# LemonATsu/UNet-PhaseGen

Hardware: AMD Instinct MI355X
Metric: spectrogram-frames/sec (train fwd+bwd) (higher is better)
Workload: dtype f32; 1 GPU; train.py full step (fwd + cos/sin/mag loss + bwd + Adam), UNetModel(1024, 2048), per-GPU batch 64 x 1024 bins x 256 frames (BASELINE configs[2]); global_batch=64, frames=256, channels=1024, parallelism=dp1, grad_allreduce_payload=fp32, adam=fused into the wgrad epilogues

## Files before the change

### unet-phasegen_amd/csrc/conv_common.h

```cpp
#pragma once
#include <hip/hip_runtime.h>
#include <stdint.h>
#include "phasegen.h"
#include "pg_common.h"

namespace pgconv {

struct IgemmParams {
    const float* x; long x_bs;
    const float* w;
    const float* pt; long pt_bs;
    float* y; long y_bs;
    const float* add; long add_bs;
    const float* ref; long ref_bs;
    unsigned x_bytes, w_bytes, pt_bytes;
    int B, Q, M, Lx, Ly, k, s, p;
    int act_x, act_p, mask_mode;
    int U, u_off;
    int LP; float inv_LP;
    int a_vec;
    int tilesM, tilesN;
    int g_ps;
    int tn_stride;
    float* y2; long y2_bs; float y_slope, y2_slope;
    float* ws;
    int nslab;
    int whole;
    int sr;
    int n_lo;
    int x_pitch;
    unsigned short* yh; long yh_bs; int yh_pitch; float yh_slope;
    unsigned short* yh2; long yh2_bs; int yh2_pitch; float yh2_slope;
    float* ad_p; float* ad_m; float* ad_v; PgAdamScalars ad;
    const float* qk; unsigned qk_bytes; int qk_bs, Lq;
    const float* pk; unsigned pk_bytes; int Kp;
};

}
using pgconv::IgemmParams;

namespace {


constexpr int WMB = 4;
constexpr int BM = 64 * WMB, BN = 128, BK = 16, NT = 256;
constexpr int TILE_A = BM * BK, TILE_B = BN * BK;
constexpr int STAGE = TILE_A + TILE_B;
constexpr int AE = BM / 16;

typedef float f32x16 __attribute__((ext_vector_type(16)));


typedef __amdgpu_buffer_rsrc_t rsrc_t;
constexpr int OOB = 0x7ffffff0;
__device__ __forceinline__ rsrc_t make_rsrc(const float* p, unsigned bytes) {
    return __builtin_amdgcn_make_buffer_rsrc(const_cast<float*>(p), 0, (int)bytes, 0x00020000);
}
__device__ __forceinline__ float bload(rsrc_t r, int elem_off, bool ok) {
    return __builtin_bit_cast(float, __builtin_amdgcn_raw_buffer_load_b32(r, ok ? elem_off * 4 : OOB, 0, 0));
}

__device__ __forceinline__ int xcd_remap(int bid, int nwg) {
    const int xcd = bid & 7, local = bid >> 3, q = nwg >> 3, r = nwg & 7;
    return (xcd < r ? xcd * (q + 1) : r * (q + 1) + (xcd - r) * q) + local;
}

template <int MB, int NB> struct AccT { f32x16 c[MB][NB]; };
using Acc = AccT<WMB, 2>;
using AccR = AccT<2, 4>;

__device__ __forceinline__ int dma_kt(int lane, int w) { return ((((lane >> 2) & 3) ^ w) << 2) | (lane & 3); }
__device__ __forceinline__ int dma_row(int lane, int w, int e) { return 16 * e + 4 * w + (lane >> 4); }

__device__ __forceinline__ int dma16_row(int lane, int w, int e) { return (4 * e + w) * 16 + (lane >> 2); }
__device__ __forceinline__ int dma16_kc(int lane) { return ((lane & 3) ^ ((lane >> 4) & 3)) << 2; }
#ifndef PG_ABL
#define PG_ABL 0
#endif
#if PG_ABL == 4
#define PG_ADDR(x) ((x) & 0x3f0)
#else
#define PG_ADDR(x) (x)
#endif
__device__ __forceinline__ void dma16(rsrc_t r, float* lds_wave_uniform, int byte_off) {
    __builtin_amdgcn_raw_ptr_buffer_load_lds(r, lds_wave_uniform, 16, PG_ADDR(byte_off), 0, 0, 0);
}
__device__ __forceinline__ void dma4(rsrc_t r, float* lds_wave_uniform, int byte_off) {
    __builtin_amdgcn_raw_ptr_buffer_load_lds(r, lds_wave_uniform, 4, PG_ADDR(byte_off), 0, 0, 0);
}
__device__ __forceinline__ void dma4s(rsrc_t r, float* lds_wave_uniform, int lane_off, int uniform_off) {
    __builtin_amdgcn_raw_ptr_buffer_load_lds(r, lds_wave_uniform, 4, lane_off, uniform_off, 0, 0);
}
__device__ __forceinline__ void dma16s(rsrc_t r, float* lds_wave_uniform, int lane_off, int uniform_off) {
    __builtin_amdgcn_raw_ptr_buffer_load_lds(r, lds_wave_uniform, 16, lane_off, uniform_off, 0, 0);
}

typedef __bf16 bf16x8 __attribute__((ext_vector_type(8)));
__device__ __forceinline__ bf16x8 to_bf16x8(float v0, float v1, float v2, float v3, float v4, float v5, float v6, float v7) {
    bf16x8 r;
    r[0] = (__bf16)v0; r[1] = (__bf16)v1; r[2] = (__bf16)v2; r[3] = (__bf16)v3;
    r[4] = (__bf16)v4; r[5] = (__bf16)v5; r[6] = (__bf16)v6; r[7] = (__bf16)v7;
    return r;
}
__device__ __forceinline__ bf16x8 to_bf16x8(const f32x4 (&v)[2]) { return to_bf16x8(v[0][0], v[0][1], v[0][2], v[0][3], v[1][0], v[1][1], v[1][2], v[1][3]); }
__device__ __forceinline__ bf16x8 to_bf16x8(const float (&v)[8]) { return to_bf16x8(v[0], v[1], v[2], v[3], v[4], v[5], v[6], v[7]); }
template <int MB, int NB>
__device__ __forceinline__ void mfma_bf16(const bf16x8 (&A)[MB], const bf16x8 (&B)[NB], AccT<MB, NB>& acc) {
#pragma unroll
    for (int i = 0; i < MB; ++i)
#pragma unroll
        for (int j = 0; j < NB; ++j) acc.c[i][j] = __builtin_amdgcn_mfma_f32_32x32x16_bf16(A[i], B[j], acc.c[i][j], 0, 0, 0);
}
typedef float f32x2 __attribute__((ext_vector_type(2)));
typedef __bf16 bf16x2 __attribute__((ext_vector_type(2)));
typedef unsigned u32x4 __attribute__((ext_vector_type(4)));
__device__ __forceinline__ void split_bf16(const float (&v)[8], bf16x8& hi, bf16x8& lo) {
    u32x4 H, L;
#pragma unroll
    for (int i = 0; i < 4; ++i) {
        const f32x2 x = {v[2 * i], v[2 * i + 1]};
        const bf16x2 h = __builtin_convertvector(x, bf16x2);
        const unsigned P = __builtin_bit_cast(unsigned, h);
// ... 363 lines not shown
```

### unet-phasegen_amd/csrc/conv_igemm.hip

```cpp
#include <hip/hip_runtime.h>
#include <cstring>
#include <cmath>
#include <algorithm>
#include "conv_fixup.h"

namespace {

constexpr int WG_PER_CU = 2;
constexpr int MAX_STREAMK_WG = 2048;
constexpr long WS_PER_WG = 2L * ACC_REGS * NT * 4;
constexpr long WS_STREAMK = (long)MAX_STREAMK_WG * WS_PER_WG;

struct Knobs {
    int prec;
    int force_mode;
    int no_raw;
    int no_tall;
    int oversub;
    int contended;
    int no_ps;
    int no_raw3;
    int all_raw3;
    int sr;
    int force_colsplit;
// ... 264 lines not shown
    if (ptrs && (!a->x || !a->w || (!a->y && !a->yh && !a->yh2))) return pg_fail(PG_ERR_NULL, "conv_fwd_h: x, w and at least one output required");
    if (((uintptr_t)a->x & 3) || ((uintptr_t)a->w & 15) || (a->x_bs & 1) || (a->x_pitch & 1))
        return pg_fail(PG_ERR_ALIGN, "conv_fwd_h: x must be 4-byte aligned with even pitch / batch stride, w 16-byte aligned");
    if (a->x_pitch <= a->Lin) return pg_fail(PG_ERR_SHAPE, "conv_fwd_h: x_pitch must exceed Lin (zero tail of at least one element)");
    if ((a->yh && a->yh_pitch < a->Lout) || (a->yh2 && a->yh2_pitch < a->Lout)) return pg_fail(PG_ERR_SHAPE, "conv_fwd_h: output pitch below Lout");
    pg_conv_args kb = {};
    kb.schedule = a->schedule;
    if (int e = decode_knobs(&kb, kn)) return e;
    p = {};
    p.x = reinterpret_cast<const float*>(a->x); p.x_bs = a->x_bs; p.x_pitch = a->x_pitch;
    p.w = reinterpret_cast<const float*>(a->w);
    p.y = a->y; p.y_bs = a->y_bs; p.y_slope = 1.0f; p.y2_slope = 1.0f;
    p.yh = a->yh; p.yh_bs = a->yh_bs; p.yh_pitch = a->yh_pitch; p.yh_slope = pg_act_slope(a->yh_act);
    p.yh2 = a->yh2; p.yh2_bs = a->yh2_bs; p.yh2_pitch = a->yh2_pitch; p.yh2_slope = pg_act_slope(a->yh2_act);
    p.B = a->B; p.Q = a->Cin; p.M = a->Cout; p.Lx = a->Lin; p.Ly = a->Lout; p.k = a->k; p.s = a->stride; p.p = a->pad;
    p.ws = (float*)a->workspace;
    const long xe = ((long)(p.B - 1) * p.x_bs + (long)p.Q * p.x_pitch) * 2;
    if (xe <= 0 || xe >= 0x7ffffff0L) return pg_fail(PG_ERR_SHAPE, "conv_fwd_h: activation tensor exceeds 2 GiB (31-bit buffer offsets)");
    p.x_bytes = (unsigned)xe;
    const int kwp = tr ? pg_shadow_taps(p.k, p.s) : p.k;
    const long wbytes = (long)p.M * (tr ? p.s : 1) * p.Q * kwp * 2;
    if (wbytes >= 0x7ffffff0L) return pg_fail(PG_ERR_SHAPE, "conv_fwd_h: weight shadow exceeds 2 GiB");
    p.w_bytes = (unsigned)wbytes;
    if (tr) {
        p.u_off = p.p / p.s;
        p.U = (p.Ly - 1 + p.p) / p.s - p.u_off + 1;
        if (p.U <= 0) return pg_fail(PG_ERR_SHAPE, "conv_fwd_h: empty output");
    }
    if (!pgconv::h_supported(tr ? KIND_T : KIND_F, p)) return pg_fail(PG_ERR_UNSUPPORTED, "conv_fwd_h: geometry not covered by the bf16-resident kernels (use the fp32-tensor entry points)");
    return PG_OK;
}

int plan_h3(const pg_convh_args* a, ConvPlan& pl) {
    Knobs kn;
    ConvPart& c = pl.main;
    IgemmParams& p = c.p;
    if (int e = h3_params(a, true, p, kn)) return e;
    const bool tr = a->transposed != 0;
    pl.kind = tr ? KIND_T : KIND_F; pl.prec = 0; pl.has_tail = false; pl.pack = 0; c.fam = FAM_H3;
    const long rows = tr ? (long)p.M * p.s : p.M, cols = (long)p.B * (tr ? p.U : p.Ly);
    p.tilesM = (int)((rows + 255) / 256);
    p.tilesN = (int)((cols + 255) / 256);
    p.tn_stride = 256;
    p.nslab = (int)((long)p.Q * (tr ? pg_shadow_taps(p.k, p.s) : p.k) / 32);
    c.tiles = (long)p.tilesM * p.tilesN;
    if (c.tiles <= 0 || c.tiles > 0x0fffffffL || p.nslab <= 0) return pg_fail(PG_ERR_SHAPE, "conv_fwd_h: empty or oversize grid");
    set_grid(c, kn, a->workspace_bytes);
    return PG_OK;
}

hipError_t launch_fixup(const ConvPlan& pl, const ConvPart& c, hipStream_t st) {
    typedef void (*Fn)(const IgemmParams, int);
#define FIX2(KIND, MB, NB, WN) {conv_fixup_kernel<KIND, MB, NB, WN, false>, conv_fixup_kernel<KIND, MB, NB, WN, true>}
    static const Fn table[4][4][2] = {
        {FIX2(FIX_F, WMB, 2, 2), FIX2(FIX_T, WMB, 2, 2), FIX2(FIX_G, WMB, 2, 2), {}},
        {FIX2(FIX_F, 2, 4, 2), FIX2(FIX_T, 2, 4, 2), FIX2(FIX_G, 2, 4, 2), FIX2(FIX_T_PM, 2, 4, 2)},
        {FIX2(FIX_F, 2, 4, 1), FIX2(FIX_T, 2, 4, 1), {}, FIX2(FIX_T_PM, 2, 4, 1)},
        {FIX2(FIX_F, 8, 2, 4), FIX2(FIX_T, 8, 2, 4), {}, {conv_fixup_kernel<FIX_T_PM, 8, 2, 4, false>, nullptr}}};
#undef FIX2
    const int geom = c.fam == FAM_IM2COL ? 0 : (c.fam == FAM_RAW_TALL ? 2 : (c.fam == FAM_RAW3 || c.fam == FAM_H3 ? 3 : 1));
    const bool pm = pl.kind == KIND_T && c.p.s == 2 && (c.fam == FAM_RAW || c.fam == FAM_RAW_TALL || c.fam == FAM_RAW3);
    const bool wide = c.fixup == FIXUP_WIDE;
    const Fn fn = table[geom][pm ? FIX_T_PM : (int)pl.kind][wide];
    if (!fn) return hipErrorInvalidDeviceFunction;
    const long blocks = (c.tiles - c.p.whole) * (geom == 3 ? 16 : 8) * (wide ? 4 : 1);
    hipLaunchKernelGGL(fn, dim3((unsigned)blocks), dim3(NT), 0, st, c.p, c.grid);
    return hipGetLastError();
}

hipError_t part_kernel(const ConvPlan& pl, const ConvPart& c, hipStream_t st, char* name = nullptr) {
    const IgemmParams& p = c.p;
    const Kind kind = pl.kind;
    const char* tk = kind == KIND_T ? "true" : "false";
    hipError_t e = hipSuccess;
    switch (c.fam) {
        case FAM_RAW_TALL:
            if (name) snprintf(name, 96, "conv_raw_kernel<%d, %d, %s, %d, 1>", p.k, p.s, tk, pl.prec);
            else e = pgconv::launch_raw_ft_tall(kind, p, c.grid, st, pl.prec);
            break;
        case FAM_RAW:
            if (name) snprintf(name, 96, "conv_raw_kernel<%d, %d, %s, %d, 2>", p.k, p.s, tk, pl.prec);
            else e = pgconv::launch_raw_ft(kind, p, c.grid, st, pl.prec);
            break;
        case FAM_G_RAW:
        case FAM_G_PS:
            if (name) snprintf(name, 96, "conv_g_%s_kernel<%d, %d, %d>", c.fam == FAM_G_PS ? "ps" : "raw", p.k, p.s, pl.prec);
            else e = pgconv::launch_raw_g(p, c.grid, st, pl.prec);
            break;
        case FAM_IM2COL:
            if (name) snprintf(name, 96, "conv_%c_kernel<0, 0, %d>", "ftg"[kind], pl.prec);
            else e = pgconv::launch_im2col(kind, p, c.grid, st, pl.prec);
            break;
        case FAM_RAW3:
            if (name) snprintf(name, 96, "conv_raw3_kernel<%d, %d, %s, %s>", p.k, p.s, tk, p.act_x == PG_ACT_NONE ? "false" : "true");
            else e = pgconv::launch_raw3(kind, p, c.grid, st);
            break;
        case FAM_H3:
            if (name) snprintf(name, 96, "conv_h3_kernel<%d, %d, %s>", kind == KIND_T && p.k == 5 ? 8 : p.k, p.s, tk);
            else e = pgconv::launch_h3(kind, p, c.grid, st);
            break;
    }
    if (!name && e == hipSuccess && c.fixup != FIXUP_NONE) e = launch_fixup(pl, c, st);
    return e;
}

void describe(const ConvPlan& pl, char* buf, int buflen) {
    static const char* const fixup_name[] = {"none", "plain", "wide"};
    const ConvPart& c = pl.main;
    char name[96];
    (void)part_kernel(pl, c, nullptr, name);
    snprintf(buf, (size_t)buflen, "%s|grid=%d|tiles=%ld|slabs=%d|split=%d|whole=%d|fixup=%s", name, c.grid, c.tiles, c.p.nslab,
             (int)(c.fixup != FIXUP_NONE), c.p.whole, fixup_name[c.fixup]);
    if (!pl.has_tail) return;
// ... 70 lines not shown
```

### unet-phasegen_amd/csrc/conv_raw_wgrad.hip

```cpp
#include "conv_common.h"

namespace {

template <int KW, int S> struct GRaw {
    static constexpr int WL = 15 * S + KW;
    static constexpr int WLP = g_wlp(KW, S);
    static constexpr int NQT = RBN / KW;
    static constexpr int TNV = NQT * KW;
    static constexpr int SUB = NQT * WLP;
    static constexpr int SUBS = (SUB + 63) / 64 * 64;
    static constexpr int NE = (SUB + NT - 1) / NT;
    static constexpr int SUBP = (SUB + 255) / 256 * 256;
    static constexpr int NE16 = (SUB / 4 + NT - 1) / NT;
    static constexpr int STG_FLAT_BF = RTILE_A + 2 * SUBS, STG_FLAT_F32 = RTILE_A + 2 * SUBP, STG_PS = RTILE_A + SUBP;
    static_assert(WL <= WLP, "window does not fit its slot");
    static_assert(WLP % 4 == 0 && WLP <= 64, "16-byte window pieces; channel 0 inside the first 64 floats");
    static_assert(2 * STG_FLAT_F32 * 4 <= 64 * 1024, "LDS budget");
};

#define G_HEAD(STG)                                                                                       \
    __shared__ __attribute__((aligned(16))) float lds[2 * (STG)];                                         \
    const int tid = threadIdx.x, lane = tid & 63;                                                         \
    const int wv = __builtin_amdgcn_readfirstlane(tid >> 6), wm = wv >> 1, wn = wv & 1;

#define G_TILE                                                                                            \
    const int m0 = (tile / p.tilesN) * RBM, n0 = (tile % p.tilesN) * C::TNV;                              \
    const int qbase = (tile % p.tilesN) * C::NQT;

#define G_A_PIECES(PITCH)                                                                                 \
    _Pragma("unroll") for (int e = 0; e < 2; ++e) {                                                       \
        const int m = m0 + dma16_row(lane, wv, e);                                                        \
        pv[e] = m < p.M ? (m * (PITCH) + dma16_kc(lane)) * 4 : FAR;                                       \
    }

#define G_FRAG_BASE_ACC(MORE)                                                                             \
    int bbase[4];                                                                                         \
    _Pragma("unroll") for (int jb = 0; jb < 4; ++jb) {                                                    \
        const int c = wn * 128 + jb * 32 + (lane & 31), qc = c / KW;                                      \
        bbase[jb] = qc * C::WLP + (c - qc * KW) + S * 8 * (lane >> 5);                                    \
        MORE                                                                                              \
    }                                                                                                     \
    AccR acc;                                                                                             \
    _Pragma("unroll") for (int i = 0; i < 2; ++i) _Pragma("unroll") for (int j = 0; j < 4; ++j)           \
        _Pragma("unroll") for (int r = 0; r < 16; ++r) acc.c[i][j][r] = 0.f;

#define G_READ_INTERIOR                                                                                   \
    _Pragma("unroll") for (int i = 0; i < 2; ++i) a[i][0] = *reinterpret_cast<const f32x4*>(ap + i * 32 * BK + (((2 * h) ^ sw) << 2)); \
    _Pragma("unroll") for (int ip = 0; ip < 4; ++ip) {                                                    \
        if (ip == 2) {                                                                                    \
            _Pragma("unroll") for (int i = 0; i < 2; ++i) a[i][1] = *reinterpret_cast<const f32x4*>(ap + i * 32 * BK + (((2 * h + 1) ^ sw) << 2)); \
        }                                                                                                 \
        _Pragma("unroll") for (int jb = 0; jb < 4; ++jb) { b[jb][2 * ip] = Bw[bbase[jb] + S * 2 * ip]; b[jb][2 * ip + 1] = Bw[bbase[jb] + S * (2 * ip + 1)]; } \
    }

#define G_READ_FLAT(SLOT)                                                                                 \
    if (kc_cur >= 16) {                                                                                   \
        G_READ_INTERIOR                                                                                   \
    } else {                                                                                              \
        _Pragma("unroll") for (int c = 0; c < 2; ++c)                                                     \
            _Pragma("unroll") for (int i = 0; i < 2; ++i) a[i][c] = *reinterpret_cast<const f32x4*>(ap + i * 32 * BK + (((2 * h + c) ^ sw) << 2)); \
        typedef const volatile __attribute__((address_space(3))) float* lds_vptr;                         \
        const lds_vptr Bv = (lds_vptr)Bw;                                                                 \
        const int shift = (SLOT) - S * kc_cur;                                                            \
        _Pragma("unroll") for (int i = 0; i < 8; ++i) {                                                   \
            const int d = (8 * h + i >= kc_cur) ? shift : 0;                                              \
            _Pragma("unroll") for (int jb = 0; jb < 4; ++jb) b[jb][i] = Bv[bbase[jb] + S * i + d];        \
        }                                                                                                 \
    }

#define G_ACT                                                                                             \
    if (slopeA != 1.0f) {                                                                                 \
        _Pragma("unroll") for (int i = 0; i < 2; ++i) _Pragma("unroll") for (int c = 0; c < 2; ++c)       \
            _Pragma("unroll") for (int v = 0; v < 4; ++v) a[i][c][v] = pg_act_apply(a[i][c][v], slopeA);  \
    }                                                                                                     \
    if (slopeB != 1.0f) {                                                                                 \
        _Pragma("unroll") for (int jb = 0; jb < 4; ++jb)                                                  \
            _Pragma("unroll") for (int i = 0; i < 8; ++i) b[jb][i] = pg_act_apply(b[jb][i], slopeB);      \
    }

#define G_MFMA(BF)                                                                                        \
    if (BF) mfma_low_2x4<BF>(a, b, acc);                                                                  \
    else {                                                                                                \
        _Pragma("unroll") for (int kk = 0; kk < 8; ++kk)                                                  \
            _Pragma("unroll") for (int i = 0; i < 2; ++i) _Pragma("unroll") for (int j = 0; j < 4; ++j)   \
                acc.c[i][j] = __builtin_amdgcn_mfma_f32_32x32x2f32(a[i][kk >> 2][kk & 3], b[j][kk], acc.c[i][j], 0, 0, 0); \
    }

#if defined(PG_G_ABL) && PG_G_ABL == 1
#define G_ISSUE_NEXT(STG, ISSUE, SKIP) SKIP
#else
#define G_ISSUE_NEXT(STG, ISSUE, SKIP) ISSUE(lds + (cur ^ 1) * (STG), (sl + 1) * BK)
#endif
#if defined(PG_G_ABL) && PG_G_ABL == 2
#define G_BARRIER asm volatile("s_waitcnt lgkmcnt(0)\n\ts_barrier" ::: "memory");
#else
#define G_BARRIER __syncthreads();
#endif

#define G_SLAB_LOOP(STG, BF, ISSUE, SKIP, PRIMED, FRAGS, ADVANCE)                                         \
    PG_STAMP_DECL                                                                                         \
    ISSUE(lds, sb * BK)                                                                                   \
    PRIMED                                                                                                \
    __syncthreads();                                                                                      \
    for (int sl = sb; sl < se; ++sl) {                                                                    \
        const int cur = (sl - sb) & 1;                                                                    \
        PG_STAMP(0)                                                                                       \
        G_ISSUE_NEXT(STG, ISSUE, SKIP)                                                                    \
        __builtin_amdgcn_sched_barrier(0);                                                                \
        PG_STAMP(1)                                                                                       \
        {   const float* As = lds + cur * (STG);                                                          \
            const float* Bw = As + RTILE_A;                                                               \
            const int r = lane & 31, h = lane >> 5, sw = (r >> 2) & 3;                                    \
            const float* ap = As + (wm * 64 + r) * BK;                                                    \
            f32x4 a[2][2];                                                                                \
            float b[4][8];                                                                                \
            FRAGS                                                                                         \
            G_MFMA(BF)                                                                                    \
        }                                                                                                 \
        __builtin_amdgcn_sched_barrier(0);                                                                \
        PG_STAMP(2)                                                                                       \
        ADVANCE                                                                                           \
        G_BARRIER                                                                                         \
        PG_STAMP(3)                                                                                       \
    }                                                                                                     \
    PG_STAMP_FLUSH

#define G_FINISH(G, SLOT)                                                                                 \
    if (sb == 0 && se == p.nslab) epilogue_g<S, 2, 4>(p, acc, m0, n0, lane, wm, wn, n0 + C::TNV);         \
    else store_partial(p.ws, G, SLOT, acc, tid);

#define G_FLAT_START                                                                                      \
    int gb, gi;                                                                                           \
    { const int k0 = sb * BK; gb = k0 / p.LP; gi = k0 - gb * p.LP; }                                      \
    int kc_cur = 16, kc_next;
#define G_FLAT_ISSUED      kc_next = kc < 16 ? kc : 16; gi += BK; if (gi >= p.LP) { gi -= p.LP; ++gb; }
#define G_FLAT_SKIP        kc_next = 16;
#define G_FLAT_ADVANCE     kc_cur = kc_next;
#define G_PS_NEXT(B_, C_)  if (++C_ == cps) { C_ = 0; ++B_; }
#define G_NOTHING

template <int KW, int S, int BF>
__device__ __forceinline__ void g_raw_bf(const IgemmParams& p) {
    using C = GRaw<KW, S>;
    G_HEAD(C::STG_FLAT_BF)
    const int kt = dma_kt(lane, wv);
    const rsrc_t rp = make_rsrc(p.pt, p.pt_bytes), rx = make_rsrc(p.x, p.x_bytes);
    const float slopeA = pg_act_slope(p.act_p), slopeB = pg_act_slope(p.act_x);
    const int pbs4 = (int)p.pt_bs * 4, xbs4 = (int)p.x_bs * 4;
    Walk wk(p);
    while (wk.more()) {
        int tile, sb, se;
        wk.segment(p, tile, sb, se);
        G_TILE

        int aoff[8];
#pragma unroll
        for (int e = 0; e < 8; ++e) {
            const int m = m0 + dma_row(lane, wv, e);
            aoff[e] = m < p.M ? m * p.LP * 4 : FAR;
        }
        constexpr bool RECOMP = KW <= 5 && BF != 0;
        int choff[RECOMP ? 1 : C::NE], vv[RECOMP ? 1 : C::NE];
        if (!RECOMP) {
#pragma unroll
            for (int e = 0; e < C::NE; ++e) {
                const int idx = tid + NT * e, ql = idx / C::WLP, v = idx - ql * C::WLP;
                choff[e] = (idx < C::SUB && qbase + ql < p.Q) ? (qbase + ql) * p.Lx * 4 : FAR;
                vv[e] = v - p.p;
            }
        }
#define GRAW_CHOFF(e) (RECOMP ? ({ int t_ = tid; asm volatile("" : "+v"(t_)); const int idx_ = t_ + NT * (e), ql_ = idx_ / C::WLP; \
                                  (idx_ < C::SUB && qbase + ql_ < p.Q) ? (qbase + ql_) * p.Lx * 4 : FAR; }) : choff[RECOMP ? 0 : (e)])
#define GRAW_VV(e) (RECOMP ? ({ int t_ = tid; asm volatile("" : "+v"(t_)); const int idx_ = t_ + NT * (e); idx_ - (idx_ / C::WLP) * C::WLP - p.p; }) \
                           : vv[RECOMP ? 0 : (e)])
        constexpr bool FASTP = BF != 2 && !(KW <= 5 && BF != 0);
        constexpr bool FASTW = FASTP && KW != 4;
        int pv[FASTP ? 2 : 1], woff[FASTW ? C::NE16 : 1];
        if (FASTW) {
#pragma unroll
            for (int e = 0; e < C::NE16; ++e) {
                const int f = 4 * (tid + NT * e), ql = f / C::WLP, v0 = f - ql * C::WLP;
                woff[e] = (f < C::SUB && qbase + ql < p.Q) ? ((qbase + ql) * p.Lx + v0) * 4 : FAR;
            }
        }
        if (FASTP) { G_A_PIECES(p.LP) }
        G_FRAG_BASE_ACC(G_NOTHING)
        G_FLAT_START

#define GRAW_ISSUE(STAGE_PTR, K0)                                                                         \
    {   float* const As = (STAGE_PTR) + wv * 64; float* const Bw = (STAGE_PTR) + RTILE_A + wv * 64;       \
        const int k0 = (K0);                                                                              \
        const int kc = p.LP - gi;                            \
        if (FASTP && kc >= 16 && gb < p.B) {                                                              \
            const int sa = gb * pbs4 + gi * 4;                                                            \
            _Pragma("unroll") for (int e = 0; e < 2; ++e) dma16s(rp, As + wv * 192 + e * 1024, pv[FASTP ? e : 0], sa); \
        } else {                                                                                          \
          int bb, ii; divmod24(k0 + kt, p.LP, p.inv_LP, bb, ii);                                          \
          const int po = bb < p.B ? bb * pbs4 + ii * 4 : OOB;                                             \
          _Pragma("unroll") for (int e = 0; e < 8; ++e) dma4(rp, As + e * 256, aoff[e] + po); }           \
        const int w0 = S * gi - p.p;                             \
        if (FASTW && kc >= 16 && gb < p.B && w0 >= 0 && w0 + C::WLP <= p.Lx) {    \
            const int sw_ = gb * xbs4 + w0 * 4;                                                           \
            _Pragma("unroll") for (int e = 0; e < C::NE16; ++e)                                           \
                if (4 * (e * NT + wv * 64) < C::SUB) dma16s(rx, (STAGE_PTR) + RTILE_A + 4 * (e * NT + wv * 64), woff[FASTW ? e : 0], sw_); \
        } else {                                                                                          \
        const int sb0 = gb < p.B ? gb * xbs4 : -NEVER, sb1 = (kc < 16 && gb + 1 < p.B) ? (gb + 1) * xbs4 : -NEVER; \
        _Pragma("unroll") for (int e = 0; e < C::NE; ++e) {                                               \
            if ((e + 1) * NT <= C::SUB || e * NT + wv * 64 < C::SUB) {                                    \
                const int ps = S * gi + GRAW_VV(e);                                                       \
                dma4(rx, Bw + e * NT, ((unsigned)ps < (unsigned)p.Lx && sb0 >= 0) ? sb0 + GRAW_CHOFF(e) + ps * 4 : FAR); \
            }                                                                                             \
        }                                                                                                 \
        if (kc < 16) {                                  \
            _Pragma("unroll") for (int e = 0; e < C::NE; ++e) {                                           \
                if ((e + 1) * NT <= C::SUB || e * NT + wv * 64 < C::SUB) {                                                          \
                    const int ps = GRAW_VV(e);                                                            \
                    dma4(rx, Bw + C::SUBS + e * NT, ((unsigned)ps < (unsigned)p.Lx && sb1 >= 0) ? sb1 + GRAW_CHOFF(e) + ps * 4 : FAR); \
                }                                                                                         \
            }                                                                                             \
        }                                                                                                 \
        }                                                                                                 \
        G_FLAT_ISSUED                                                                                     \
    }
#define GRAW_FRAGS G_READ_FLAT(C::SUBS) G_ACT
        G_SLAB_LOOP(C::STG_FLAT_BF, BF, GRAW_ISSUE, G_FLAT_SKIP, G_FLAT_ADVANCE, GRAW_FRAGS, G_FLAT_ADVANCE)
#undef GRAW_FRAGS
#undef GRAW_ISSUE
#undef GRAW_CHOFF
#undef GRAW_VV
        G_FINISH(wk.g, wk.slot)
        wk.next(se - sb);
    }
}

template <int KW, int S, int BF>
__device__ __forceinline__ void g_ps_bf(const IgemmParams& p) {
    using C = GRaw<KW, S>;
    G_HEAD(C::STG_PS)
    const rsrc_t rp = make_rsrc(p.pt, p.pt_bytes), rx = make_rsrc(p.x, p.x_bytes);
    const float slopeA = pg_act_slope(p.act_p), slopeB = pg_act_slope(p.act_x);
    const int pbs4 = (int)p.pt_bs * 4, xbs4 = (int)p.x_bs * 4;
    const int cps = (p.LP + 15) >> 4;
    Walk wk(p);
    while (wk.more()) {
        int tile, sb, se;
        wk.segment(p, tile, sb, se);
        G_TILE

        int pv[2], woff[C::NE16];
        G_A_PIECES(p.LP)
#pragma unroll
        for (int e = 0; e < C::NE16; ++e) {
            const int f = 4 * (tid + NT * e), ql = f / C::WLP, v0 = f - ql * C::WLP;
            const int off = ((qbase + ql) * p.Lx + v0 - p.p) * 4;
            woff[e] = (f < C::SUB && qbase + ql < p.Q && off >= 0) ? off : FAR;
        }
        const bool fix0 = qbase == 0 && wv == 0;
        int f0_off, f0_v;
        { const int ql = lane / C::WLP, v = lane - ql * C::WLP; f0_off = ql < p.Q ? ql * p.Lx * 4 : FAR; f0_v = v - p.p; }
        int pj[4];
#define GPS_PJ pj[jb] = (c - qc * KW) + S * 8 * (lane >> 5) - p.p;
        G_FRAG_BASE_ACC(GPS_PJ)
#undef GPS_PJ

        int gb = sb / cps, gc = sb - gb * cps;
        int mc = gc;
#define GPS_ISSUE(STAGE_PTR, K0)                                                                          \
    {   float* const As = (STAGE_PTR) + wv * 64;                                                          \
        if (gb < p.B) {                                                                                   \
            const int gi = gc << 4;                                                                       \
            const int sa = gb * pbs4 + gi * 4;                                                            \
            _Pragma("unroll") for (int e = 0; e < 2; ++e) dma16s(rp, As + wv * 192 + e * 1024, pv[e], sa); \
            const int sw_ = gb * xbs4 + S * gi * 4;                                                       \
            _Pragma("unroll") for (int e = 0; e < C::NE16; ++e)                                           \
                if (4 * (e * NT + wv * 64) < C::SUB) dma16s(rx, (STAGE_PTR) + RTILE_A + 4 * (e * NT + wv * 64), woff[e], sw_); \
            if (fix0) {                                                                                   \
                const int ps = S * gi + f0_v;                                                             \
                dma4(rx, (STAGE_PTR) + RTILE_A, (unsigned)ps < (unsigned)p.Lx ? gb * xbs4 + f0_off + ps * 4 : FAR); \
            }                                                                                             \
        }                                                                                                 \
        G_PS_NEXT(gb, gc)                                                                                 \
    }
#define GPS_FRAGS                                                                                         \
    const int gi = mc << 4, kc = p.LP - gi;                   \
    const int w0 = S * gi;                                \
    G_READ_INTERIOR                                                                                       \
    if (kc < 16) {                           \
        _Pragma("unroll") for (int i = 0; i < 2; ++i) _Pragma("unroll") for (int c = 0; c < 2; ++c)       \
            _Pragma("unroll") for (int v = 0; v < 4; ++v) a[i][c][v] = (8 * h + 4 * c + v < kc) ? a[i][c][v] : 0.f; \
    }                                                                                                     \
    if (w0 < p.p || w0 - p.p + C::WLP > p.Lx) {    \
        _Pragma("unroll") for (int jb = 0; jb < 4; ++jb)                                                  \
            _Pragma("unroll") for (int i = 0; i < 8; ++i) b[jb][i] = (unsigned)(w0 + pj[jb] + S * i) < (unsigned)p.Lx ? b[jb][i] : 0.f; \
    }                                                                                                     \
    G_ACT
#define GPS_ADVANCE if (++mc == cps) mc = 0;
        G_SLAB_LOOP(C::STG_PS, BF, GPS_ISSUE, G_NOTHING, G_NOTHING, GPS_FRAGS, GPS_ADVANCE)
#undef GPS_ADVANCE
#undef GPS_FRAGS
#undef GPS_ISSUE
        G_FINISH(wk.g, wk.slot)
        wk.next(se - sb);
    }
}

template <int KW, int S>
__device__ __forceinline__ void g_raw_f32(const IgemmParams& p) {
    using C = GRaw<KW, S>;
    constexpr int NP = 2 * C::SUBP / 4;
    constexpr int NE2 = (NP + NT - 1) / NT;
    G_HEAD(C::STG_FLAT_F32)
    const rsrc_t rp = make_rsrc(p.pk, p.pk_bytes), rx = make_rsrc(p.qk, p.qk_bytes);
    const int qbs4 = p.qk_bs * 4, klast4 = (p.nslab - 1) * BK * 4;
    Walk wk(p);
    while (wk.more()) {
        int tile, sb, se;
        wk.segment(p, tile, sb, se);
        G_TILE
        int pv[2], woff[NE2];
        G_A_PIECES(p.Kp)
#pragma unroll
        for (int e = 0; e < NE2; ++e) {
            const int pc = tid + NT * e, sub = pc >= C::SUBP / 4 ? 1 : 0, f = 4 * pc - sub * C::SUBP, ql = f / C::WLP, v0 = f - ql * C::WLP;
            woff[e] = (f < C::SUB && qbase + ql < p.Q) ? ((qbase + ql) * p.Lq + v0) * 4 : FAR;
        }
        G_FRAG_BASE_ACC(G_NOTHING)
        G_FLAT_START
#define GRF_ISSUE(STAGE_PTR, K0)                                                                          \
    {   const int sa = min((K0) * 4, klast4);                                                             \
        _Pragma("unroll") for (int e = 0; e < 2; ++e) dma16s(rp, (STAGE_PTR) + wv * 256 + e * 1024, pv[e], sa); \
        const int kc = p.LP - gi;                                                                         \
        const int sw0 = min(gb, p.B - 1) * qbs4 + S * gi * 4;                                             \
        const int sw1 = (kc < 16 && gb + 1 < p.B) ? (gb + 1) * qbs4 : sw0;                                \
        _Pragma("unroll") for (int e = 0; e < NE2; ++e) {                                                 \
            const int pc0 = e * NT + wv * 64;                                 \
            if ((e + 1) * NT <= NP || pc0 < NP)                                                           \
                dma16s(rx, (STAGE_PTR) + RTILE_A + 4 * pc0, woff[e], pc0 >= C::SUBP / 4 ? sw1 : sw0);     \
        }                                                                                                 \
        G_FLAT_ISSUED                                                                                     \
    }
#define GRF_FRAGS G_READ_FLAT(C::SUBP)
        G_SLAB_LOOP(C::STG_FLAT_F32, 0, GRF_ISSUE, G_FLAT_SKIP, G_FLAT_ADVANCE, GRF_FRAGS, G_FLAT_ADVANCE)
#undef GRF_FRAGS
#undef GRF_ISSUE
        G_FINISH(wk.g, wk.slot)
        wk.next(se - sb);
    }
}

template <int KW, int S>
__device__ __forceinline__ void g_ps_f32(const IgemmParams& p) {
    using C = GRaw<KW, S>;
    G_HEAD(C::STG_PS)
    const rsrc_t rp = make_rsrc(p.pk, p.pk_bytes), rx = make_rsrc(p.qk, p.qk_bytes);
    const int pbs4 = p.M * p.Kp * 4, qbs4 = p.qk_bs * 4;
    const int cps = p.Kp >> 4;
    const int g = logical_wg(blockIdx.x, gridDim.x, p.whole);
    const Split sp = make_split(p.tilesM * p.tilesN, p.nslab, gridDim.x, p.whole);
    int pos = split_lo(sp, g);
    const int pos_end = split_lo(sp, g + 1);
    int slot = 0;
    while (pos < pos_end) {
        const int tile = pos / p.nslab, sb = pos - tile * p.nslab;
        const int se = min(p.nslab, sb + (pos_end - pos));
        G_TILE
        int pv[2], woff[C::NE16];
        G_A_PIECES(p.Kp)
#pragma unroll
        for (int e = 0; e < C::NE16; ++e) {
            const int f = 4 * (tid + NT * e), ql = f / C::WLP, v0 = f - ql * C::WLP;
            woff[e] = (f < C::SUB && qbase + ql < p.Q) ? ((qbase + ql) * p.Lq + v0) * 4 : FAR;
        }
        G_FRAG_BASE_ACC(G_NOTHING)

        int gb = sb / cps, gc = sb - gb * cps;
#define GPF_ISSUE(STAGE_PTR, K0)                                                                          \
    {   const int gbc = min(gb, p.B - 1), gi = gc << 4;                                                   \
        _Pragma("unroll") for (int e = 0; e < 2; ++e) dma16s(rp, (STAGE_PTR) + wv * 256 + e * 1024, pv[e], gbc * pbs4 + gi * 4); \
        const int sw_ = gbc * qbs4 + S * gi * 4;                                                          \
        _Pragma("unroll") for (int e = 0; e < C::NE16; ++e)                                               \
            if (4 * (e * NT + wv * 64) < C::SUB) dma16s(rx, (STAGE_PTR) + RTILE_A + 4 * (e * NT + wv * 64), woff[e], sw_); \
        G_PS_NEXT(gb, gc)                                                                                 \
    }
        G_SLAB_LOOP(C::STG_PS, 0, GPF_ISSUE, G_NOTHING, G_NOTHING, G_READ_INTERIOR, G_NOTHING)
#undef GPF_ISSUE
        G_FINISH(g, slot)
        pos += se - sb;
        slot = 1;
    }
}

template <int KW, int S, int BF>
__global__ __launch_bounds__(NT, 2) void conv_g_raw_kernel(const IgemmParams p) {
    if constexpr (BF == 0) g_raw_f32<KW, S>(p);
    else g_raw_bf<KW, S, BF>(p);
}
template <int KW, int S, int BF>
__global__ __launch_bounds__(NT, 2) void conv_g_ps_kernel(const IgemmParams p) {
    if constexpr (BF == 0) g_ps_f32<KW, S>(p);
    else g_ps_bf<KW, S, BF>(p);
}

__global__ __launch_bounds__(256) void pack_rows_kernel(const float* __restrict__ src, long bs, int C, int L, int F, int W, unsigned n,
                                                       float slope, float* __restrict__ dst) {
    for (unsigned i = blockIdx.x * 256u + threadIdx.x; i < n; i += gridDim.x * 256u) {
        const unsigned r = i / (unsigned)W, b = r / (unsigned)C, c = r - b * (unsigned)C;
        const int t = (int)(i - r * (unsigned)W) - F;
        float v = 0.f;
        if ((unsigned)t < (unsigned)L) {
            v = src[(long)b * bs + (long)c * L + t];
            if (slope != 1.0f) v = pg_act_apply(v, slope);
        }
        dst[i] = v;
    }
}
__global__ __launch_bounds__(256) void pack_flat_kernel(const float* __restrict__ src, long bs, int B, int LP, int Kp, unsigned n,
                                                       float slope, float* __restrict__ dst) {
    for (unsigned i = blockIdx.x * 256u + threadIdx.x; i < n; i += gridDim.x * 256u) {
        const unsigned m = i / (unsigned)Kp, k = i - m * (unsigned)Kp, b = k / (unsigned)LP, t = k - b * (unsigned)LP;
        float v = 0.f;
        if ((int)b < B) {
            v = src[(long)b * bs + (long)m * LP + t];
            if (slope != 1.0f) v = pg_act_apply(v, slope);
        }
        dst[i] = v;
    }
}
unsigned pack_grid(unsigned n) { return (n + 255u) / 256u < 2048u ? (n + 255u) / 256u : 2048u; }

hipError_t pack_g(const IgemmParams& p, hipStream_t st) {
    float* const qk = const_cast<float*>(p.qk);
    float* const pk = const_cast<float*>(p.pk);
    const unsigned nq = (unsigned)(p.qk_bytes / 4), np = (unsigned)(p.pk_bytes / 4);
    hipLaunchKernelGGL(pack_rows_kernel, dim3(pack_grid(nq)), dim3(256), 0, st, p.x, p.x_bs, p.Q, p.Lx, p.p, p.Lq, nq, pg_act_slope(p.act_x), qk);
    if (p.g_ps) hipLaunchKernelGGL(pack_rows_kernel, dim3(pack_grid(np)), dim3(256), 0, st, p.pt, p.pt_bs, p.M, p.LP, 0, p.Kp, np, pg_act_slope(p.act_p), pk);
    else hipLaunchKernelGGL(pack_flat_kernel, dim3(pack_grid(np)), dim3(256), 0, st, p.pt, p.pt_bs, p.B, p.LP, p.Kp, np, pg_act_slope(p.act_p), pk);
    return hipGetLastError();
}

typedef void (*g_kernel_t)(const IgemmParams);
template <int KW, int S, int BF> g_kernel_t g_kernel(bool ps) { return ps ? conv_g_ps_kernel<KW, S, BF> : conv_g_raw_kernel<KW, S, BF>; }

template <int KW, int S>
hipError_t launch_g_raw(const IgemmParams& p, int grid, hipStream_t st, int prec) {
    if (prec == 0) {
        if (hipError_t e = pack_g(p, st)) return e;
    }
    const g_kernel_t kernel = prec == 1 ? g_kernel<KW, S, 1>(p.g_ps) : (prec == 2 ? g_kernel<KW, S, 2>(p.g_ps) : g_kernel<KW, S, 0>(p.g_ps));
    hipLaunchKernelGGL(kernel, dim3(grid), dim3(NT), 0, st, p);
    return hipGetLastError();
}

}

hipError_t pgconv::launch_raw_g(const IgemmParams& p, int grid, hipStream_t st, int prec) {
    if (p.k == 32) return launch_g_raw<32, 2>(p, grid, st, prec);
    if (p.k == 8 && p.s == 1) return launch_g_raw<8, 1>(p, grid, st, prec);
    if (p.k == 8) return launch_g_raw<8, 2>(p, grid, st, prec);
    if (p.k == 5) return launch_g_raw<5, 2>(p, grid, st, prec);
    return launch_g_raw<4, 2>(p, grid, st, prec);
}
```

Measured before the change: 98990 frames/s.

## Reshape fp32 wgrad warp tiling to 4x2 and vectorize pack kernels

The fp32 weight-gradient kernels now give each wave a 4x2 block of MFMA tiles (all four waves split along N) instead of 2x4, which changes how many A and B fragments each wave reads from LDS per MFMA. A matching fixup table entry is added for that geometry. The pack kernels that stage activations into padded rows are rewritten to use 2D/3D grids with float4 loads and stores and several rows per thread, replacing per-element index division. This raises register pressure per wave and adds alignment-dependent branches.

```diff
diff --git a/unet-phasegen_amd/csrc/conv_common.h b/unet-phasegen_amd/csrc/conv_common.h
--- a/unet-phasegen_amd/csrc/conv_common.h
+++ b/unet-phasegen_amd/csrc/conv_common.h
@@ -68,6 +68,11 @@
 template <int MB, int NB> struct AccT { f32x16 c[MB][NB]; };
 using Acc = AccT<WMB, 2>;
 using AccR = AccT<2, 4>;
+#if defined(PG_G_ABL) && PG_G_ABL == 3
+#define G_F32_MB 2
+#else
+#define G_F32_MB 4
+#endif
 
 __device__ __forceinline__ int dma_kt(int lane, int w) { return ((((lane >> 2) & 3) ^ w) << 2) | (lane & 3); }
 __device__ __forceinline__ int dma_row(int lane, int w, int e) { return 16 * e + 4 * w + (lane >> 4); }
diff --git a/unet-phasegen_amd/csrc/conv_igemm.hip b/unet-phasegen_amd/csrc/conv_igemm.hip
--- a/unet-phasegen_amd/csrc/conv_igemm.hip
+++ b/unet-phasegen_amd/csrc/conv_igemm.hip
@@ -340,13 +340,15 @@
 hipError_t launch_fixup(const ConvPlan& pl, const ConvPart& c, hipStream_t st) {
     typedef void (*Fn)(const IgemmParams, int);
 #define FIX2(KIND, MB, NB, WN) {conv_fixup_kernel<KIND, MB, NB, WN, false>, conv_fixup_kernel<KIND, MB, NB, WN, true>}
-    static const Fn table[4][4][2] = {
+    static const Fn table[5][4][2] = {
         {FIX2(FIX_F, WMB, 2, 2), FIX2(FIX_T, WMB, 2, 2), FIX2(FIX_G, WMB, 2, 2), {}},
         {FIX2(FIX_F, 2, 4, 2), FIX2(FIX_T, 2, 4, 2), FIX2(FIX_G, 2, 4, 2), FIX2(FIX_T_PM, 2, 4, 2)},
         {FIX2(FIX_F, 2, 4, 1), FIX2(FIX_T, 2, 4, 1), {}, FIX2(FIX_T_PM, 2, 4, 1)},
-        {FIX2(FIX_F, 8, 2, 4), FIX2(FIX_T, 8, 2, 4), {}, {conv_fixup_kernel<FIX_T_PM, 8, 2, 4, false>, nullptr}}};
+        {FIX2(FIX_F, 8, 2, 4), FIX2(FIX_T, 8, 2, 4), {}, {conv_fixup_kernel<FIX_T_PM, 8, 2, 4, false>, nullptr}},
+        {{}, {}, FIX2(FIX_G, G_F32_MB, 8 / G_F32_MB, G_F32_MB == 4 ? 4 : 2), {}}};
 #undef FIX2
-    const int geom = c.fam == FAM_IM2COL ? 0 : (c.fam == FAM_RAW_TALL ? 2 : (c.fam == FAM_RAW3 || c.fam == FAM_H3 ? 3 : 1));
+    const bool g32 = (c.fam == FAM_G_RAW || c.fam == FAM_G_PS) && pl.prec == 0;
+    const int geom = c.fam == FAM_IM2COL ? 0 : (c.fam == FAM_RAW_TALL ? 2 : (c.fam == FAM_RAW3 || c.fam == FAM_H3 ? 3 : (g32 ? 4 : 1)));
     const bool pm = pl.kind == KIND_T && c.p.s == 2 && (c.fam == FAM_RAW || c.fam == FAM_RAW_TALL || c.fam == FAM_RAW3);
     const bool wide = c.fixup == FIXUP_WIDE;
     const Fn fn = table[geom][pm ? FIX_T_PM : (int)pl.kind][wide];
diff --git a/unet-phasegen_amd/csrc/conv_raw_wgrad.hip b/unet-phasegen_amd/csrc/conv_raw_wgrad.hip
--- a/unet-phasegen_amd/csrc/conv_raw_wgrad.hip
+++ b/unet-phasegen_amd/csrc/conv_raw_wgrad.hip
@@ -18,10 +18,11 @@
     static_assert(2 * STG_FLAT_F32 * 4 <= 64 * 1024, "LDS budget");
 };
 
-#define G_HEAD(STG)                                                                                       \
+#define G_HEAD(STG, MB_)                                                                                  \
     __shared__ __attribute__((aligned(16))) float lds[2 * (STG)];                                         \
+    constexpr int MB = (MB_), NB = 8 / MB;                                                                \
     const int tid = threadIdx.x, lane = tid & 63;                                                         \
-    const int wv = __builtin_amdgcn_readfirstlane(tid >> 6), wm = wv >> 1, wn = wv & 1;
+    const int wv = __builtin_amdgcn_readfirstlane(tid >> 6), wm = MB == 2 ? wv >> 1 : 0, wn = MB == 2 ? wv & 1 : wv;
 
 #define G_TILE                                                                                            \
     const int m0 = (tile / p.tilesN) * RBM, n0 = (tile % p.tilesN) * C::TNV;                              \
@@ -34,23 +35,23 @@
     }
 
 #define G_FRAG_BASE_ACC(MORE)                                                                             \
-    int bbase[4];                                                                                         \
-    _Pragma("unroll") for (int jb = 0; jb < 4; ++jb) {                                                    \
-        const int c = wn * 128 + jb * 32 + (lane & 31), qc = c / KW;                                      \
+    int bbase[NB];                                                                                        \
+    _Pragma("unroll") for (int jb = 0; jb < NB; ++jb) {                                                   \
+        const int c = wn * (NB * 32) + jb * 32 + (lane & 31), qc = c / KW;                                \
         bbase[jb] = qc * C::WLP + (c - qc * KW) + S * 8 * (lane >> 5);                                    \
         MORE                                                                                              \
     }                                                                                                     \
-    AccR acc;                                                                                             \
-    _Pragma("unroll") for (int i = 0; i < 2; ++i) _Pragma("unroll") for (int j = 0; j < 4; ++j)           \
+    AccT<MB, NB> acc;                                                                                     \
+    _Pragma("unroll") for (int i = 0; i < MB; ++i) _Pragma("unroll") for (int j = 0; j < NB; ++j)         \
         _Pragma("unroll") for (int r = 0; r < 16; ++r) acc.c[i][j][r] = 0.f;
 
 #define G_READ_INTERIOR                                                                                   \
-    _Pragma("unroll") for (int i = 0; i < 2; ++i) a[i][0] = *reinterpret_cast<const f32x4*>(ap + i * 32 * BK + (((2 * h) ^ sw) << 2)); \
+    _Pragma("unroll") for (int i = 0; i < MB; ++i) a[i][0] = *reinterpret_cast<const f32x4*>(ap + i * 32 * BK + (((2 * h) ^ sw) << 2)); \
     _Pragma("unroll") for (int ip = 0; ip < 4; ++ip) {                                                    \
         if (ip == 2) {                                                                                    \
-            _Pragma("unroll") for (int i = 0; i < 2; ++i) a[i][1] = *reinterpret_cast<const f32x4*>(ap + i * 32 * BK + (((2 * h + 1) ^ sw) << 2)); \
-        }                                                                                                 \
-        _Pragma("unroll") for (int jb = 0; jb < 4; ++jb) { b[jb][2 * ip] = Bw[bbase[jb] + S * 2 * ip]; b[jb][2 * ip + 1] = Bw[bbase[jb] + S * (2 * ip + 1)]; } \
+            _Pragma("unroll") for (int i = 0; i < MB; ++i) a[i][1] = *reinterpret_cast<const f32x4*>(ap + i * 32 * BK + (((2 * h + 1) ^ sw) << 2)); \
+        }                                                                                                 \
+        _Pragma("unroll") for (int jb = 0; jb < NB; ++jb) { b[jb][2 * ip] = Bw[bbase[jb] + S * 2 * ip]; b[jb][2 * ip + 1] = Bw[bbase[jb] + S * (2 * ip + 1)]; } \
     }
 
 #define G_READ_FLAT(SLOT)                                                                                 \
@@ -58,33 +59,31 @@
         G_READ_INTERIOR                                                                                   \
     } else {                                                                                              \
         _Pragma("unroll") for (int c = 0; c < 2; ++c)                                                     \
-            _Pragma("unroll") for (int i = 0; i < 2; ++i) a[i][c] = *reinterpret_cast<const f32x4*>(ap + i * 32 * BK + (((2 * h + c) ^ sw) << 2)); \
+            _Pragma("unroll") for (int i = 0; i < MB; ++i) a[i][c] = *reinterpret_cast<const f32x4*>(ap + i * 32 * BK + (((2 * h + c) ^ sw) << 2)); \
         typedef const volatile __attribute__((address_space(3))) float* lds_vptr;                         \
         const lds_vptr Bv = (lds_vptr)Bw;                                                                 \
         const int shift = (SLOT) - S * kc_cur;                                                            \
         _Pragma("unroll") for (int i = 0; i < 8; ++i) {                                                   \
             const int d = (8 * h + i >= kc_cur) ? shift : 0;                                              \
-            _Pragma("unroll") for (int jb = 0; jb < 4; ++jb) b[jb][i] = Bv[bbase[jb] + S * i + d];        \
+            _Pragma("unroll") for (int jb = 0; jb < NB; ++jb) b[jb][i] = Bv[bbase[jb] + S * i + d];       \
         }                                                                                                 \
     }
 
 #define G_ACT                                                                                             \
     if (slopeA != 1.0f) {                                                                                 \
-        _Pragma("unroll") for (int i = 0; i < 2; ++i) _Pragma("unroll") for (int c = 0; c < 2; ++c)       \
+        _Pragma("unroll") for (int i = 0; i < MB; ++i) _Pragma("unroll") for (int c = 0; c < 2; ++c)      \
             _Pragma("unroll") for (int v = 0; v < 4; ++v) a[i][c][v] = pg_act_apply(a[i][c][v], slopeA);  \
     }                                                                                                     \
     if (slopeB != 1.0f) {                                                                                 \
-        _Pragma("unroll") for (int jb = 0; jb < 4; ++jb)                                                  \
+        _Pragma("unroll") for (int jb = 0; jb < NB; ++jb)                                                 \
             _Pragma("unroll") for (int i = 0; i < 8; ++i) b[jb][i] = pg_act_apply(b[jb][i], slopeB);      \
     }
 
-#define G_MFMA(BF)                                                                                        \
-    if (BF) mfma_low_2x4<BF>(a, b, acc);                                                                  \
-    else {                                                                                                \
-        _Pragma("unroll") for (int kk = 0; kk < 8; ++kk)                                                  \
-            _Pragma("unroll") for (int i = 0; i < 2; ++i) _Pragma("unroll") for (int j = 0; j < 4; ++j)   \
-                acc.c[i][j] = __builtin_amdgcn_mfma_f32_32x32x2f32(a[i][kk >> 2][kk & 3], b[j][kk], acc.c[i][j], 0, 0, 0); \
-    }
+#define G_MFMA_F32                                                                                        \
+    _Pragma("unroll") for (int kk = 0; kk < 8; ++kk)                                                      \
+        _Pragma("unroll") for (int i = 0; i < MB; ++i) _Pragma("unroll") for (int j = 0; j < NB; ++j)     \
+            acc.c[i][j] = __builtin_amdgcn_mfma_f32_32x32x2f32(a[i][kk >> 2][kk & 3], b[j][kk], acc.c[i][j], 0, 0, 0);
+#define G_MFMA_LOW mfma_low_2x4<BF>(a, b, acc);
 
 #if defined(PG_G_ABL) && PG_G_ABL == 1
 #define G_ISSUE_NEXT(STG, ISSUE, SKIP) SKIP
@@ -97,7 +96,7 @@
 #define G_BARRIER __syncthreads();
 #endif
 
-#define G_SLAB_LOOP(STG, BF, ISSUE, SKIP, PRIMED, FRAGS, ADVANCE)                                         \
+#define G_SLAB_LOOP(STG, MFMA, ISSUE, SKIP, PRIMED, FRAGS, ADVANCE)                                         \
     PG_STAMP_DECL                                                                                         \
     ISSUE(lds, sb * BK)                                                                                   \
     PRIMED                                                                                                \
@@ -111,11 +110,11 @@
         {   const float* As = lds + cur * (STG);                                                          \
             const float* Bw = As + RTILE_A;                                                               \
             const int r = lane & 31, h = lane >> 5, sw = (r >> 2) & 3;                                    \
-            const float* ap = As + (wm * 64 + r) * BK;                                                    \
-            f32x4 a[2][2];                                                                                \
-            float b[4][8];                                                                                \
+            const float* ap = As + (wm * (MB * 32) + r) * BK;                                             \
+            f32x4 a[MB][2];                                                                               \
+            float b[NB][8];                                                                               \
             FRAGS                                                                                         \
-            G_MFMA(BF)                                                                                    \
+            MFMA                                                                                          \
         }                                                                                                 \
         __builtin_amdgcn_sched_barrier(0);                                                                \
         PG_STAMP(2)                                                                                       \
@@ -126,7 +125,7 @@
     PG_STAMP_FLUSH
 
 #define G_FINISH(G, SLOT)                                                                                 \
-    if (sb == 0 && se == p.nslab) epilogue_g<S, 2, 4>(p, acc, m0, n0, lane, wm, wn, n0 + C::TNV);         \
+    if (sb == 0 && se == p.nslab) epilogue_g<S, MB, NB>(p, acc, m0, n0, lane, wm, wn, n0 + C::TNV);       \
     else store_partial(p.ws, G, SLOT, acc, tid);
 
 #define G_FLAT_START                                                                                      \
@@ -142,7 +141,7 @@
 template <int KW, int S, int BF>
 __device__ __forceinline__ void g_raw_bf(const IgemmParams& p) {
     using C = GRaw<KW, S>;
-    G_HEAD(C::STG_FLAT_BF)
+    G_HEAD(C::STG_FLAT_BF, 2)
     const int kt = dma_kt(lane, wv);
     const rsrc_t rp = make_rsrc(p.pt, p.pt_bytes), rx = make_rsrc(p.x, p.x_bytes);
     const float slopeA = pg_act_slope(p.act_p), slopeB = pg_act_slope(p.act_x);
@@ -223,7 +222,7 @@
         G_FLAT_ISSUED                                                                                     \
     }
 #define GRAW_FRAGS G_READ_FLAT(C::SUBS) G_ACT
-        G_SLAB_LOOP(C::STG_FLAT_BF, BF, GRAW_ISSUE, G_FLAT_SKIP, G_FLAT_ADVANCE, GRAW_FRAGS, G_FLAT_ADVANCE)
+        G_SLAB_LOOP(C::STG_FLAT_BF, G_MFMA_LOW, GRAW_ISSUE, G_FLAT_SKIP, G_FLAT_ADVANCE, GRAW_FRAGS, G_FLAT_ADVANCE)
 #undef GRAW_FRAGS
 #undef GRAW_ISSUE
 #undef GRAW_CHOFF
@@ -236,7 +235,7 @@
 template <int KW, int S, int BF>
 __device__ __forceinline__ void g_ps_bf(const IgemmParams& p) {
     using C = GRaw<KW, S>;
-    G_HEAD(C::STG_PS)
+    G_HEAD(C::STG_PS, 2)
     const rsrc_t rp = make_rsrc(p.pt, p.pt_bytes), rx = make_rsrc(p.x, p.x_bytes);
     const float slopeA = pg_act_slope(p.act_p), slopeB = pg_act_slope(p.act_x);
     const int pbs4 = (int)p.pt_bs * 4, xbs4 = (int)p.x_bs * 4;
@@ -286,16 +285,16 @@
     const int w0 = S * gi;                                \
     G_READ_INTERIOR                                                                                       \
     if (kc < 16) {                           \
-        _Pragma("unroll") for (int i = 0; i < 2; ++i) _Pragma("unroll") for (int c = 0; c < 2; ++c)       \
+        _Pragma("unroll") for (int i = 0; i < MB; ++i) _Pragma("unroll") for (int c = 0; c < 2; ++c)      \
             _Pragma("unroll") for (int v = 0; v < 4; ++v) a[i][c][v] = (8 * h + 4 * c + v < kc) ? a[i][c][v] : 0.f; \
     }                                                                                                     \
     if (w0 < p.p || w0 - p.p + C::WLP > p.Lx) {    \
-        _Pragma("unroll") for (int jb = 0; jb < 4; ++jb)                                                  \
+        _Pragma("unroll") for (int jb = 0; jb < NB; ++jb)                                                 \
             _Pragma("unroll") for (int i = 0; i < 8; ++i) b[jb][i] = (unsigned)(w0 + pj[jb] + S * i) < (unsigned)p.Lx ? b[jb][i] : 0.f; \
     }                                                                                                     \
     G_ACT
 #define GPS_ADVANCE if (++mc == cps) mc = 0;
-        G_SLAB_LOOP(C::STG_PS, BF, GPS_ISSUE, G_NOTHING, G_NOTHING, GPS_FRAGS, GPS_ADVANCE)
+        G_SLAB_LOOP(C::STG_PS, G_MFMA_LOW, GPS_ISSUE, G_NOTHING, G_NOTHING, GPS_FRAGS, GPS_ADVANCE)
 #undef GPS_ADVANCE
 #undef GPS_FRAGS
 #undef GPS_ISSUE
@@ -309,7 +308,7 @@
     using C = GRaw<KW, S>;
     constexpr int NP = 2 * C::SUBP / 4;
     constexpr int NE2 = (NP + NT - 1) / NT;
-    G_HEAD(C::STG_FLAT_F32)
+    G_HEAD(C::STG_FLAT_F32, G_F32_MB)
     const rsrc_t rp = make_rsrc(p.pk, p.pk_bytes), rx = make_rsrc(p.qk, p.qk_bytes);
     const int qbs4 = p.qk_bs * 4, klast4 = (p.nslab - 1) * BK * 4;
     Walk wk(p);
@@ -340,7 +339,7 @@
         G_FLAT_ISSUED                                                                                     \
     }
 #define GRF_FRAGS G_READ_FLAT(C::SUBP)
-        G_SLAB_LOOP(C::STG_FLAT_F32, 0, GRF_ISSUE, G_FLAT_SKIP, G_FLAT_ADVANCE, GRF_FRAGS, G_FLAT_ADVANCE)
+        G_SLAB_LOOP(C::STG_FLAT_F32, G_MFMA_F32, GRF_ISSUE, G_FLAT_SKIP, G_FLAT_ADVANCE, GRF_FRAGS, G_FLAT_ADVANCE)
 #undef GRF_FRAGS
 #undef GRF_ISSUE
         G_FINISH(wk.g, wk.slot)
@@ -351,7 +350,7 @@
 template <int KW, int S>
 __device__ __forceinline__ void g_ps_f32(const IgemmParams& p) {
     using C = GRaw<KW, S>;
-    G_HEAD(C::STG_PS)
+    G_HEAD(C::STG_PS, G_F32_MB)
     const rsrc_t rp = make_rsrc(p.pk, p.pk_bytes), rx = make_rsrc(p.qk, p.qk_bytes);
     const int pbs4 = p.M * p.Kp * 4, qbs4 = p.qk_bs * 4;
     const int cps = p.Kp >> 4;
@@ -382,7 +381,7 @@
             if (4 * (e * NT + wv * 64) < C::SUB) dma16s(rx, (STAGE_PTR) + RTILE_A + 4 * (e * NT + wv * 64), woff[e], sw_); \
         G_PS_NEXT(gb, gc)                                                                                 \
     }
-        G_SLAB_LOOP(C::STG_PS, 0, GPF_ISSUE, G_NOTHING, G_NOTHING, G_READ_INTERIOR, G_NOTHING)
+        G_SLAB_LOOP(C::STG_PS, G_MFMA_F32, GPF_ISSUE, G_NOTHING, G_NOTHING, G_READ_INTERIOR, G_NOTHING)
 #undef GPF_ISSUE
         G_FINISH(g, slot)
         pos += se - sb;
@@ -401,40 +400,110 @@
     else g_ps_bf<KW, S, BF>(p);
 }
 
-__global__ __launch_bounds__(256) void pack_rows_kernel(const float* __restrict__ src, long bs, int C, int L, int F, int W, unsigned n,
+constexpr int PACK_ROWS = 4, PACK_FLAT_ROWS = 8;
+
+__global__ __launch_bounds__(256) void pack_rows_kernel(const float* __restrict__ src, long bs, int B, int C, int L, int F, int W,
+                                                       bool v4, float slope, float* __restrict__ dst) {
+    const int c0 = blockIdx.x * (blockDim.y * PACK_ROWS) + threadIdx.y;
+    for (int b = blockIdx.z; b < B; b += gridDim.z) {
+        const float* sb = src + (long)b * bs;
+        float* db = dst + (long)b * C * W;
+        for (int j = (blockIdx.y * blockDim.x + threadIdx.x) * 4; j < W; j += gridDim.y * blockDim.x * 4) {
+            const int t0 = j - F;
+            const bool inside = t0 >= 0 && t0 + 3 < L;
+            f32x4 v[PACK_ROWS];
+#pragma unroll
+            for (int e = 0; e < PACK_ROWS; ++e) {
+                const int c = c0 + e * blockDim.y;
+                v[e] = f32x4{0.f, 0.f, 0.f, 0.f};
+                if (c >= C) continue;
+                const float* s = sb + (long)c * L + t0;
+                if (inside && (reinterpret_cast<uintptr_t>(s) & 15) == 0) v[e] = *reinterpret_cast<const f32x4*>(s);
+                else {
+#pragma unroll
+                    for (int q = 0; q < 4; ++q)
+                        if ((unsigned)(t0 + q) < (unsigned)L) v[e][q] = s[q];
+                }
+            }
+#pragma unroll
+            for (int e = 0; e < PACK_ROWS; ++e) {
+                const int c = c0 + e * blockDim.y;
+                if (c >= C) continue;
+                if (slope != 1.0f) {
+#pragma unroll
+                    for (int q = 0; q < 4; ++q) v[e][q] = pg_act_apply(v[e][q], slope);
+                }
+                float* d = db + (long)c * W + j;
+                if (v4) *reinterpret_cast<f32x4*>(d) = v[e];
+                else {
+#pragma unroll
+                    for (int q = 0; q < 4; ++q)
+                        if (j + q < W) d[q] = v[e][q];
+                }
+            }
+        }
+    }
+}
+__global__ __launch_bounds__(256) void pack_flat_kernel(const float* __restrict__ src, long bs, int M, int B, int LP, int Kp, bool v4,
                                                        float slope, float* __restrict__ dst) {
-    for (unsigned i = blockIdx.x * 256u + threadIdx.x; i < n; i += gridDim.x * 256u) {
-        const unsigned r = i / (unsigned)W, b = r / (unsigned)C, c = r - b * (unsigned)C;
-        const int t = (int)(i - r * (unsigned)W) - F;
-        float v = 0.f;
-        if ((unsigned)t < (unsigned)L) {
-            v = src[(long)b * bs + (long)c * L + t];
-            if (slope != 1.0f) v = pg_act_apply(v, slope);
-        }
-        dst[i] = v;
-    }
-}
-__global__ __launch_bounds__(256) void pack_flat_kernel(const float* __restrict__ src, long bs, int B, int LP, int Kp, unsigned n,
-                                                       float slope, float* __restrict__ dst) {
-    for (unsigned i = blockIdx.x * 256u + threadIdx.x; i < n; i += gridDim.x * 256u) {
-        const unsigned m = i / (unsigned)Kp, k = i - m * (unsigned)Kp, b = k / (unsigned)LP, t = k - b * (unsigned)LP;
-        float v = 0.f;
-        if ((int)b < B) {
-            v = src[(long)b * bs + (long)m * LP + t];
-            if (slope != 1.0f) v = pg_act_apply(v, slope);
-        }
-        dst[i] = v;
-    }
-}
-unsigned pack_grid(unsigned n) { return (n + 255u) / 256u < 2048u ? (n + 255u) / 256u : 2048u; }
+    const unsigned k0 = (blockIdx.x * 256u + threadIdx.x) * 4u;
+    if (k0 >= (unsigned)Kp) return;
+    long off[4];
+    {
+        unsigned b = k0 / (unsigned)LP, t = k0 - b * (unsigned)LP;
+#pragma unroll
+        for (int q = 0; q < 4; ++q) {
+            off[q] = b < (unsigned)B ? (long)b * bs + t : -1;
+            if (++t == (unsigned)LP) { t = 0; ++b; }
+        }
+    }
+    for (int m0 = blockIdx.y * PACK_FLAT_ROWS; m0 < M; m0 += gridDim.y * PACK_FLAT_ROWS) {
+        f32x4 v[PACK_FLAT_ROWS];
+#pragma unroll
+        for (int e = 0; e < PACK_FLAT_ROWS; ++e) {
+            v[e] = f32x4{0.f, 0.f, 0.f, 0.f};
+            if (m0 + e >= M) continue;
+            const float* s = src + (long)(m0 + e) * LP;
+#pragma unroll
+            for (int q = 0; q < 4; ++q)
+                if (off[q] >= 0) v[e][q] = s[off[q]];
+        }
+#pragma unroll
+        for (int e = 0; e < PACK_FLAT_ROWS; ++e) {
+            if (m0 + e >= M) continue;
+            if (slope != 1.0f) {
+#pragma unroll
+                for (int q = 0; q < 4; ++q) v[e][q] = pg_act_apply(v[e][q], slope);
+            }
+            float* d = dst + (long)(m0 + e) * Kp + k0;
+            if (v4) *reinterpret_cast<f32x4*>(d) = v[e];
+            else {
+#pragma unroll
+                for (int q = 0; q < 4; ++q) d[q] = v[e][q];
+            }
+        }
+    }
+}
+
+bool pack_v4(const float* dst, int W) { return W % 4 == 0 && (reinterpret_cast<uintptr_t>(dst) & 15) == 0; }
+unsigned pack_dim(long n) { return (unsigned)(n < 65535 ? n : 65535); }
+
+void launch_pack_rows(const float* src, long bs, int B, int C, int L, int F, int W, float slope, float* dst, hipStream_t st) {
+    const int n4 = (W + 3) / 4;
+    int tx = 4;
+    while (tx < 256 && tx < n4) tx *= 2;
+    const int ty = 256 / tx, cb = ty * PACK_ROWS;
+    hipLaunchKernelGGL(pack_rows_kernel, dim3((C + cb - 1) / cb, pack_dim((n4 + tx - 1) / tx), pack_dim(B)), dim3(tx, ty), 0, st, src, bs, B, C,
+                       L, F, W, pack_v4(dst, W), slope, dst);
+}
 
 hipError_t pack_g(const IgemmParams& p, hipStream_t st) {
     float* const qk = const_cast<float*>(p.qk);
     float* const pk = const_cast<float*>(p.pk);
-    const unsigned nq = (unsigned)(p.qk_bytes / 4), np = (unsigned)(p.pk_bytes / 4);
-    hipLaunchKernelGGL(pack_rows_kernel, dim3(pack_grid(nq)), dim3(256), 0, st, p.x, p.x_bs, p.Q, p.Lx, p.p, p.Lq, nq, pg_act_slope(p.act_x), qk);
-    if (p.g_ps) hipLaunchKernelGGL(pack_rows_kernel, dim3(pack_grid(np)), dim3(256), 0, st, p.pt, p.pt_bs, p.M, p.LP, 0, p.Kp, np, pg_act_slope(p.act_p), pk);
-    else hipLaunchKernelGGL(pack_flat_kernel, dim3(pack_grid(np)), dim3(256), 0, st, p.pt, p.pt_bs, p.B, p.LP, p.Kp, np, pg_act_slope(p.act_p), pk);
+    launch_pack_rows(p.x, p.x_bs, p.B, p.Q, p.Lx, p.p, p.Lq, pg_act_slope(p.act_x), qk, st);
+    if (p.g_ps) launch_pack_rows(p.pt, p.pt_bs, p.B, p.M, p.LP, 0, p.Kp, pg_act_slope(p.act_p), pk, st);
+    else hipLaunchKernelGGL(pack_flat_kernel, dim3((p.Kp + 1023) / 1024, pack_dim((p.M + PACK_FLAT_ROWS - 1) / PACK_FLAT_ROWS)), dim3(256), 0, st,
+                            p.pt, p.pt_bs, p.M, p.B, p.LP, p.Kp, pack_v4(pk, p.Kp), pg_act_slope(p.act_p), pk);
     return hipGetLastError();
 }
 
```

Result: no change. 99260 frames/s, median of 6 (+0.3%).
